# kcat/openal-soft

Measured on AMD Instinct MI355X. Metric: mixed voices/sec @48kHz 1024-sample update, HRTF stereo; fraction of HBM roofline, higher is better.
Workload: dtype f32

## Files before the change

include/oalgpu.h:

```cpp
#ifndef OALGPU_H
#define OALGPU_H

#include <stddef.h>
#include <stdint.h>

#ifdef __cplusplus
extern "C" {
#endif
#if defined(__GNUC__)
#pragma GCC visibility push(default)
#endif

#define OALGPU_BUFFER_LINE_SIZE 1024
#define OALGPU_MAX_RESAMPLER_PADDING 48
#define OALGPU_MAX_RESAMPLER_EDGE 24
#define OALGPU_HRTF_HISTORY_LENGTH 64
#define OALGPU_HRIR_LENGTH 128
#define OALGPU_MAX_SENDS 6
#define OALGPU_MAX_OUTPUT_CHANNELS 32
#define OALGPU_MAX_AMBI_CHANNELS 25
#define OALGPU_MIXER_FRAC_BITS 16

typedef enum oalgpu_error {
    OALGPU_OK = 0,
// ... 47 lines not shown
    float sf;
    uint32_t m, l;
    uint32_t filter_offset;
} oalgpu_interp_state;
int oalgpu_prepare_resampler(int resampler, uint32_t increment, oalgpu_interp_state *out);

typedef struct oalgpu_biquad {
    float z1, z2;
    float b0, b1, b2, a1, a2;
    float tb0, tb1, tb2, ta1, ta2;
    int32_t counter;
} oalgpu_biquad;
void oalgpu_biquad_reset(oalgpu_biquad *f);
void oalgpu_biquad_set_params_from_slope(oalgpu_biquad *f, int type, float f0norm, float gain,
    float slope);

int oalgpu_resample(int device, int mode, int resampler, uint32_t increment, const float *src,
    size_t srclen, uint32_t frac, float *dst, size_t n);
int oalgpu_mix(int device, const float *in, size_t n, float *out, size_t nlines,
    float *current_gains, const float *target_gains, size_t counter, size_t outpos);
int oalgpu_mix_hrtf(int device, int mode, const float *in, float *accum, uint32_t irsize,
    const float *coeffs, const uint32_t delay[2], float gain, float gainstep, size_t n);
int oalgpu_mix_hrtf_blend(int device, int mode, const float *in, float *accum, uint32_t irsize,
    const float *oldcoeffs, const uint32_t olddelay[2], float oldgain, const float *newcoeffs,
    const uint32_t newdelay[2], float newgainstep, size_t n);
typedef struct oalgpu_splitter { float coeff, lp_z1, lp_z2, ap_z1; } oalgpu_splitter;
void oalgpu_splitter_init(oalgpu_splitter *s, float f0norm);
int oalgpu_mix_direct_hrtf(int device, int mode, float *left, float *right, const float *in,
    size_t nch, float *accum, oalgpu_splitter *splitters, const float *hfscales,
    const float *chan_coeffs, size_t irsize, size_t n);
int oalgpu_biquad_dual_process(int device, oalgpu_biquad *f0, oalgpu_biquad *f1, const float *src,
    float *dst, size_t n);

typedef struct oalgpu_context oalgpu_context;

typedef struct oalgpu_context_desc {
    int32_t  device;
    int32_t  math_mode;
    uint32_t sample_rate;
    uint32_t num_dry_channels;
    uint32_t num_real_channels;
    uint32_t num_aux_sends;
    uint32_t num_slots;
    uint32_t wet_channels;
    int32_t  hrtf;
    uint32_t max_voices;
    uint32_t max_buffers;
    uint32_t voices_per_group;
    uint32_t flags;
} oalgpu_context_desc;
#define OALGPU_CTX_FIR_VALU 1u
#define OALGPU_CTX_PROFILE  2u
#define OALGPU_CTX_STREAM_ROWS 8u
#define OALGPU_CTX_APPLY_IN_VOICE_KERNEL 16u
#define OALGPU_CTX_FUSED_REDUCE 32u
#define OALGPU_CTX_RESIDENT 64u
#define OALGPU_CTX_SLICE_LINES 128u
#define OALGPU_CTX_WAVE_PAIRS 256u
#define OALGPU_CTX_ROW_SLICES 512u
#define OALGPU_CTX_SERIAL   4u

int  oalgpu_context_create(const oalgpu_context_desc *desc, oalgpu_context **out);
void oalgpu_context_destroy(oalgpu_context *ctx);

int oalgpu_hrtf_load_mhr(oalgpu_context *ctx, const void *data, size_t size);
int oalgpu_hrtf_load_store(oalgpu_context *ctx, uint32_t sample_rate, uint32_t ir_size, const float *field_distance,
    const uint8_t *field_evcount, uint32_t num_fields, const uint16_t *elev_azcount, const uint16_t *elev_iroffset,
    uint32_t num_elevs, const float *coeffs, const uint8_t *delays, uint32_t num_irs);
typedef struct oalgpu_hrtf_info {
    uint32_t sample_rate, ir_size, num_fields, num_elevs, num_irs;
} oalgpu_hrtf_info;
int oalgpu_hrtf_info_get(oalgpu_context *ctx, oalgpu_hrtf_info *out);
int oalgpu_hrtf_raw(oalgpu_context *ctx, float *field_distance, uint8_t *field_evcount,
    uint16_t *elev_azcount, uint16_t *elev_iroffset, float *coeffs, uint8_t *delays);
int oalgpu_hrtf_get_coeffs(oalgpu_context *ctx, const float *dirs, size_t count, float *coeffs,
    uint32_t *delays);
int oalgpu_set_direct_hrtf(oalgpu_context *ctx, const float *chan_coeffs ,
    const float *hfscales, float xover_norm, uint32_t irsize);
int oalgpu_set_direct_hrtf_from_store(oalgpu_context *ctx, const float *points, const float *matrix, uint32_t num_points,
    const float *order_hf_gain, float xover_freq, uint32_t ir_size, int per_hrir_min);
int oalgpu_hrtf_parse_host(const void *mhr, size_t size, uint32_t device_rate, oalgpu_hrtf_info *info, float *coeffs, uint8_t *delays);
int oalgpu_hrtf_blend_host(const void *mhr, size_t size, uint32_t device_rate, const float *dirs, size_t count,
    uint32_t *idx, float *w, float *pass, uint32_t *delays);
int oalgpu_hrtf_build_direct_host(const void *mhr, size_t size, uint32_t device_rate, uint32_t ir_size, int per_hrir_min,
    const float *points, const float *matrix, uint32_t num_points, uint32_t num_chans, float xover_freq, const float *order_hf_gain,
    float *out_coeffs, float *out_hfscales, float *out_xover_norm, uint32_t *out_irsize);

int oalgpu_buffer_register(oalgpu_context *ctx, const void *data, int fmt_type,
    uint32_t frame_step, uint32_t sample_len, uint32_t loop_start, uint32_t loop_end);
int oalgpu_buffer_release(oalgpu_context *ctx, int buffer);
int oalgpu_buffer_info(oalgpu_context *ctx, int buffer, int32_t *live, int32_t *release_pending, uint32_t *references);

int oalgpu_buffer_channel_view(oalgpu_context *ctx, int buffer, uint32_t channel);

typedef struct oalgpu_voice_desc {
    int32_t  buffer;
    int32_t  looping;
    int32_t  position;
    uint32_t position_frac;
    uint32_t frequency;
} oalgpu_voice_desc;
int oalgpu_voice_init(oalgpu_context *ctx, uint32_t voice, const oalgpu_voice_desc *desc);
int oalgpu_context_set_nfc(oalgpu_context *ctx, float w1, const uint32_t channels_per_order[5]);
int oalgpu_voice_set_nfc(oalgpu_context *ctx, uint32_t voice, float w0);

int oalgpu_voice_set_ambi_scale(oalgpu_context *ctx, uint32_t voice, float xover_norm, float hf_scale,
    float lf_scale);

typedef struct oalgpu_filter_params {
    int32_t active;
    float gain_hf, hf_norm;
    float gain_lf, lf_norm;
} oalgpu_filter_params;

typedef struct oalgpu_voice_params {
    uint32_t step;
    int32_t  resampler;
    oalgpu_filter_params direct_filter;
    float    dry_gains[OALGPU_MAX_OUTPUT_CHANNELS];
    float    hrtf_ev, hrtf_az, hrtf_dist, hrtf_spread;
    float    hrtf_gain;
    int32_t  send_slot[OALGPU_MAX_SENDS];
    oalgpu_filter_params send_filter[OALGPU_MAX_SENDS];
    float    send_gains[OALGPU_MAX_SENDS][OALGPU_MAX_AMBI_CHANNELS];
} oalgpu_voice_params;
#define OALGPU_HRTF_KEEP_TARGET (-1.0f)
int oalgpu_voice_set_hrtf_targets(oalgpu_context *ctx, const uint32_t *voices, const float *coeffs, const uint32_t *delays,
    const float *gains, size_t count);

typedef struct oalgpu_voice_pan {
    float dir[3];
    float spread;
    float dry_gain;
    float send_gain[OALGPU_MAX_SENDS];
} oalgpu_voice_pan;
int oalgpu_context_set_ambi_map(oalgpu_context *ctx, const uint8_t *index, const float *scale);
int oalgpu_slot_set_ambi_map(oalgpu_context *ctx, uint32_t slot, const uint8_t *index, const float *scale);
int oalgpu_voice_set_pan(oalgpu_context *ctx, const uint32_t *voices, const oalgpu_voice_pan *pans, size_t count);

int oalgpu_buffer_queue_link(oalgpu_context *ctx, int buffer, int next_buffer);
int oalgpu_voice_init_queue(oalgpu_context *ctx, uint32_t voice, int first_buffer, int looping, int32_t position,
    uint32_t position_frac);
int oalgpu_voice_queue_state(oalgpu_context *ctx, uint32_t voice, int32_t *current_buffer, uint32_t *buffers_done);
int oalgpu_voice_queue_unqueue(oalgpu_context *ctx, uint32_t voice, uint32_t count);

typedef int32_t (*oalgpu_callback_fn)(void *userptr, void *data, int32_t num_bytes);
int oalgpu_voice_init_callback(oalgpu_context *ctx, uint32_t voice, int fmt_type, uint32_t position_frac,
    oalgpu_callback_fn fn, void *userptr);
typedef struct oalgpu_callback_state {
    int32_t position;
    uint32_t position_frac, num_blocks, block_offset;
    int32_t stopped, play_state, has_buffer;
} oalgpu_callback_state;
int oalgpu_voice_callback_state(oalgpu_context *ctx, uint32_t voice, oalgpu_callback_state *out);

enum oalgpu_adpcm_type { OALGPU_ADPCM_IMA4 = 0, OALGPU_ADPCM_MS = 1 };
int oalgpu_buffer_register_adpcm(oalgpu_context *ctx, const void *data, int adpcm_type, uint32_t channels,
    uint32_t samples_per_block, uint32_t sample_len, uint32_t loop_start, uint32_t loop_end);

int oalgpu_voice_set_start_delay(oalgpu_context *ctx, uint32_t voice, uint32_t samples);

int oalgpu_voice_set_params(oalgpu_context *ctx, const uint32_t *voices,
    const oalgpu_voice_params *params, size_t count);
typedef struct oalgpu_param_block oalgpu_param_block;
int  oalgpu_param_block_create(oalgpu_context *ctx, const uint32_t *voices,
    const oalgpu_voice_params *params, size_t count, oalgpu_param_block **out);
// ... 329 lines not shown
```

openal-soft_amd/csrc/api_hrtf.hip:

```cpp
#include "api_context.hpp"

static uint32_t ChooseWave16(const oalgpu_context *c, const DeviceLayout &T)
{
    const bool want16 = !(c->desc.flags & OALGPU_CTX_WAVE_PAIRS) && Wave16Applies(T)
        && (T.numSends == 0 || !(c->desc.flags & (OALGPU_CTX_STREAM_ROWS | OALGPU_CTX_PROFILE)));
    if(!want16) return 0u;
    if(!c->desc.voices_per_group) return Wave16WavesFor(T.numVoices, DeviceComputeUnits(c->desc.device));
    for(uint32_t w : {4u, 8u, 16u})
        if((T.numVoices + w - 1u) / w <= c->groupsAllocated) return w;
    return 0u;
}

static int InstallHrtfData(oalgpu_context *c, HrtfData &&parsed)
{
    if(parsed.sampleRate != c->desc.sample_rate) ResampleHrtfData(parsed, c->desc.sample_rate);
    DeviceLayout T = c->L;
    T.irSize = parsed.irSize;
    T.irStride = (parsed.irSize + 15u) & ~15u;
    const bool toStreamRows = T.accLines && WaveKernelAccLines(T) == 0;
    if(toStreamRows) T.accLines = 0;
    if(c->useWave)
    {
        T.wave16 = ChooseWave16(c, T);
        if(std::max<uint32_t>(1u, WaveKernelGroups(T)) > c->groupsAllocated)
            return Fail(OALGPU_ERR_INVALID, "internal: the voice kernel's grid outgrew the partial buses");
    }
    if(int rc = oalgpu_sync(c)) return rc;
    c->hrtfHost = std::move(parsed);
    const HrtfData &h = c->hrtfHost;
    HIP_TRY(c->hFieldDist.alloc(h.fieldDistance.size())); HIP_TRY(c->hFieldDist.upload(h.fieldDistance.data(), h.fieldDistance.size()));
    HIP_TRY(c->hEvCount.alloc(h.fieldEvCount.size())); HIP_TRY(c->hEvCount.upload(h.fieldEvCount.data(), h.fieldEvCount.size()));
    HIP_TRY(c->hAzCount.alloc(h.elevAzCount.size())); HIP_TRY(c->hAzCount.upload(h.elevAzCount.data(), h.elevAzCount.size()));
    HIP_TRY(c->hIrOffset.alloc(h.elevIrOffset.size())); HIP_TRY(c->hIrOffset.upload(h.elevIrOffset.data(), h.elevIrOffset.size()));
    HIP_TRY(c->hCoeffs.alloc(h.coeffs.size())); HIP_TRY(c->hCoeffs.upload(h.coeffs.data(), h.coeffs.size()));
    HIP_TRY(c->hDelays.alloc(h.delays.size())); HIP_TRY(c->hDelays.upload(h.delays.data(), h.delays.size()));
    HrtfStoreDev &d = c->hrtfDev;
    d.irSize = h.irSize; d.numFields = uint32_t(h.fieldDistance.size()); d.numElevs = uint32_t(h.elevAzCount.size());
    d.numIrs = h.numIrs();
    d.fieldDistance = c->hFieldDist.p; d.fieldEvCount = c->hEvCount.p; d.elevAzCount = c->hAzCount.p;
    d.elevIrOffset = c->hIrOffset.p; d.coeffs = c->hCoeffs.p; d.delays = c->hDelays.p;
    c->hrtfLoaded = true;
    ++c->hrtfGeneration;

    DeviceLayout &L = c->L;
    L.hrirs = c->hCoeffs.p;
    L.irSize = h.irSize;
    L.irStride = T.irStride;
    if(L.hrtf)
    {
        const size_t n = size_t{L.numVoices} * L.irStride * 2;
        HIP_TRY(c->hrtfOld.alloc(n)); HIP_TRY(c->hrtfOld.zero()); L.hrtfOld = c->hrtfOld.p;
        HIP_TRY(c->hrtfTgt.alloc(n)); HIP_TRY(c->hrtfTgt.zero()); L.hrtfTgt = c->hrtfTgt.p;
        if(!c->directSet) c->dIrSize = h.irSize;
    }
    if(toStreamRows)
    {
        L.accLines = 0;
        if(int rc = AllocStreamRows(c)) return rc;
    }
    if(c->useWave)
    {
        L.wave16 = T.wave16;
        if(L.wave16 && L.numSends)
        {
            L.accLines = 0;
            if(!L.streams) { if(int rc = AllocStreamRows(c)) return rc; }
        }
        const uint32_t groups = std::max<uint32_t>(1u, WaveKernelGroups(L));
        L.numGroups = groups; L.numLineGroups = groups;
        if(L.wave16 && (L.wave16 != 16u || L.numSends)) c->res.enabled = false;
    }
    return OALGPU_OK;
}

int oalgpu_hrtf_load_mhr(oalgpu_context *c, const void *data, size_t size)
{
    if(!c || !data) return Fail(OALGPU_ERR_INVALID, "null argument");
    if(int rc = UseCtx(c)) return rc;
    HrtfData parsed;
    const std::string err = ParseMhr(data, size, parsed);
    if(!err.empty()) return Fail(OALGPU_ERR_INVALID, "mhr: " + err);
    return InstallHrtfData(c, std::move(parsed));
}
// ... 73 lines not shown
}

int oalgpu_set_direct_hrtf(oalgpu_context *c, const float *chan_coeffs, const float *hfscales, float xover_norm,
    uint32_t irsize)
{
    if(!c || !chan_coeffs || !hfscales || irsize < 8 || irsize > kHrirLen) return Fail(OALGPU_ERR_INVALID, "oalgpu_set_direct_hrtf: bad arguments");
    if(int rc = UseCtx(c)) return rc;
    const uint32_t nd = c->L.numDry;
    std::vector<SplitterState> sp(nd);
    for(auto &s : sp) { s.coeff = SplitterCoeff(xover_norm); s.lpZ1 = s.lpZ2 = s.apZ1 = 0.0f; }
    if(int rc = oalgpu_sync(c)) return rc;
    HIP_TRY(c->dSplit.upload(sp.data(), nd));
    HIP_TRY(c->dSplit2.upload(sp.data(), nd));
    c->dSplitCur = 0;
    c->dSplitCoeff = SplitterCoeff(xover_norm); c->runPowerSeg = 0;
    HIP_TRY(c->dHfScale.upload(hfscales, nd));
    {
        std::vector<float> cc(chan_coeffs, chan_coeffs + size_t{nd} * kHrirLen * 2);
        const uint32_t live = (irsize + 1u) & ~1u;
        for(uint32_t ch = 0; ch < nd; ++ch)
            for(uint32_t k = live; k < uint32_t(kHrirLen); ++k) { cc[(size_t{ch} * kHrirLen + k) * 2] = 0.0f; cc[(size_t{ch} * kHrirLen + k) * 2 + 1] = 0.0f; }
        HIP_TRY(c->dCoeffs.upload(cc.data(), cc.size()));
    }
    c->dIrSize = irsize;
    c->directSet = true;
    return OALGPU_OK;
}

int oalgpu_set_direct_hrtf_from_store(oalgpu_context *c, const float *points, const float *matrix, uint32_t num_points,
    const float *order_hf_gain, float xover_freq, uint32_t ir_size, int per_hrir_min)
{
    if(!c || !points || !matrix || !order_hf_gain || num_points == 0 || c->L.numDry > 16)
        return Fail(OALGPU_ERR_INVALID, "oalgpu_set_direct_hrtf_from_store: bad arguments");
    if(!c->hrtfLoaded) return Fail(OALGPU_ERR_NO_HRTF, "oalgpu_set_direct_hrtf_from_store: no data set loaded");
    const DirectHrtfBuild b = BuildDirectHrtf(c->hrtfHost, ir_size ? ir_size : c->hrtfHost.irSize, per_hrir_min != 0, points, matrix,
        num_points, c->L.numDry, xover_freq, order_hf_gain);
    return oalgpu_set_direct_hrtf(c, b.coeffs.data(), b.hfScale.data(), b.xoverNorm, std::max<uint32_t>(b.irSize, 8u));
}

int oalgpu_hrtf_parse_host(const void *mhr, size_t size, uint32_t device_rate, oalgpu_hrtf_info *info, float *coeffs, uint8_t *delays)
{
    if(!mhr || !info) return Fail(OALGPU_ERR_INVALID, "null argument");
    HrtfData h;
    const std::string err = ParseMhr(mhr, size, h);
    if(!err.empty()) return Fail(OALGPU_ERR_INVALID, "mhr: " + err);
    if(device_rate) ResampleHrtfData(h, device_rate);
    info->sample_rate = h.sampleRate; info->ir_size = h.irSize; info->num_fields = uint32_t(h.fieldDistance.size());
    info->num_elevs = uint32_t(h.elevAzCount.size()); info->num_irs = h.numIrs();
    if(coeffs) std::memcpy(coeffs, h.coeffs.data(), h.coeffs.size() * sizeof(float));
    if(delays) std::memcpy(delays, h.delays.data(), h.delays.size());
    return OALGPU_OK;
}

HrtfStoreDev HostStoreView(const HrtfData &h)
{
    HrtfStoreDev st{};
    st.irSize = h.irSize; st.numFields = uint32_t(h.fieldDistance.size());
    st.numElevs = uint32_t(h.elevAzCount.size()); st.numIrs = h.numIrs();
    st.fieldDistance = h.fieldDistance.data(); st.fieldEvCount = h.fieldEvCount.data();
    st.elevAzCount = h.elevAzCount.data(); st.elevIrOffset = h.elevIrOffset.data();
    st.coeffs = h.coeffs.data(); st.delays = h.delays.data();
    return st;
}

int oalgpu_hrtf_blend_host(const void *mhr, size_t size, uint32_t device_rate, const float *dirs, size_t count,
    uint32_t *idx, float *w, float *pass, uint32_t *delays)
{
    if(!mhr || !dirs || !idx || !w || !pass || !delays) return Fail(OALGPU_ERR_INVALID, "null argument");
    HrtfData h;
    const std::string err = ParseMhr(mhr, size, h);
    if(!err.empty()) return Fail(OALGPU_ERR_INVALID, "mhr: " + err);
    if(device_rate) ResampleHrtfData(h, device_rate);
    const HrtfStoreDev store = HostStoreView(h);
    for(size_t i = 0; i < count; ++i)
    {
        const HrirBlend b = HrtfBlendFor(store, dirs[4 * i], dirs[4 * i + 1], dirs[4 * i + 2], dirs[4 * i + 3]);
        for(int k = 0; k < 4; ++k) { idx[4 * i + k] = b.idx[k]; w[4 * i + k] = b.w[k]; }
        pass[i] = b.passthru;
        delays[2 * i] = b.delay[0]; delays[2 * i + 1] = b.delay[1];
    }
    return OALGPU_OK;
}

int oalgpu_hrtf_build_direct_host(const void *mhr, size_t size, uint32_t device_rate, uint32_t ir_size, int per_hrir_min,
    const float *points, const float *matrix, uint32_t num_points, uint32_t num_chans, float xover_freq, const float *order_hf_gain,
    float *out_coeffs, float *out_hfscales, float *out_xover_norm, uint32_t *out_irsize)
{
    if(!mhr || !points || !matrix || !order_hf_gain || !out_coeffs || !out_hfscales || num_chans < 1 || num_chans > 16 || num_points == 0)
        return Fail(OALGPU_ERR_INVALID, "oalgpu_hrtf_build_direct_host: bad arguments");
    HrtfData h;
    const std::string err = ParseMhr(mhr, size, h);
    if(!err.empty()) return Fail(OALGPU_ERR_INVALID, "mhr: " + err);
    if(device_rate) ResampleHrtfData(h, device_rate);
    const DirectHrtfBuild b = BuildDirectHrtf(h, ir_size ? ir_size : h.irSize, per_hrir_min != 0, points, matrix, num_points,
        num_chans, xover_freq, order_hf_gain);
    std::memcpy(out_coeffs, b.coeffs.data(), b.coeffs.size() * sizeof(float));
    std::memcpy(out_hfscales, b.hfScale.data(), b.hfScale.size() * sizeof(float));
    if(out_xover_norm) *out_xover_norm = b.xoverNorm;
    if(out_irsize) *out_irsize = b.irSize;
    return OALGPU_OK;
}
```

openal-soft_amd/csrc/voice_wave16.hip:

```cpp
#define OALGPU_WAVE_NO_LAUNCHER
#include "voice_wave.hip"

#pragma clang fp contract(off)

namespace oalgpu {
namespace {

constexpr int kW16Outs = kLine / 64;

constexpr int kW16Rd = 1184;
constexpr int kW16Rd2 = kMaxEdge + kPre * 64 + 8;
constexpr int kW16Area = kResampleDataSize + kLine;
static_assert(kW16Rd % 64 == 32 && kW16Rd >= kMaxPad + kPre * 64 + 8, "rd2 sits half the banks away from rd");
static_assert(kW16Rd + kW16Rd2 <= kW16Area, "the twice-parked window fits");
static_assert(kResampleDataSize >= kLine + 64, "a send's filter scan parks the unfiltered samples in the window's area");
constexpr int kW16DumpF2 = 64 * 17 + 68;
static_assert(kW16DumpF2 * 2 <= kW16Area, "the dump fits");
struct W16PhaseB {
    uint32_t xh[2][kXhDw];
    uint32_t hr[2][kHrDw];
    uint32_t hro[2][kHrDw];
    float in0[2 * kHist];
};
static_assert(sizeof(W16PhaseB) <= size_t(kW16Area) * 4, "phase B fits the area (nothing of it is written before the sample line is back in registers)");
struct alignas(16) W16Lds {
    union {
        struct { float rd[kW16Rd]; float rd2[kW16Rd2]; } a;
        struct { float rd[kResampleDataSize]; float smp[kLine]; } g;
        W16PhaseB b;
        f2 dump[kW16DumpF2];
        float raw[kW16Area];
    };
    int32_t best;
    uint32_t pad[3];
};
template<int WAVES>
struct W16Wg {
    alignas(16) f2 tabF[12 * 32];
    f2 tabP[12 * 32];
    uint32_t tabKey, tabM, tabL, pad;
    uint32_t res[12];
    W16Lds w[WAVES];
};
static_assert(sizeof(W16Wg<16>) <= 157440, "123 LDS granules: the post-process (4) and the reduction (1) fit beside it");

struct W16GenView { float *rd, *in, *rd2; int32_t &best; uint32_t *pad; };

template<int M, bool DUAL>
__device__ __forceinline__ void ResampleRingRegs(const f2 *tabF, const f2 *tabP, const float *rdb, uint32_t frac0, uint32_t increment,
    uint32_t bdst, float (&outs)[kW16Outs], uint32_t lane, const float *rd2b, uint32_t rdbIndex)
{
    constexpr int NP = (M / 2 >= 6) ? 6 : M / 2;
    constexpr int G = (M / 2) / NP;
    f2 F[2][NP], P[2][NP], S[2][NP];
    const uint32_t tstep = 64u * increment;
    const uint32_t tlast = frac0 + (bdst - 1u) * increment;
    auto load = [&](int set, uint32_t tt, int g)
    {
        tt = tt < tlast ? tt : tlast;
        const uint32_t pi = (tt >> 11) & 31u;
        const f2 *tf = tabF + pi, *tp = tabP + pi;
        const uint32_t pos = tt >> kFracBits;
#pragma unroll
        for(int q = 0; q < NP; ++q)
        {
            F[set][q] = tf[(g * NP + q) * 32];
            P[set][q] = tp[(g * NP + q) * 32];
        }
        if constexpr (DUAL)
        {
            const bool odd = ((rdbIndex + pos) & 1u) != 0u;
            const f2 *sp = reinterpret_cast<const f2*>(odd ? rd2b + pos - 1u : rdb + pos);
#pragma unroll
            for(int q = 0; q < NP; ++q) S[set][q] = sp[g * NP + q];
        }
        else
        {
            const float *s = rdb + pos;
#pragma unroll
            for(int q = 0; q < NP; ++q) S[set][q] = f2{s[2 * (g * NP + q)], s[2 * (g * NP + q) + 1]};
        }
    };
    const uint32_t tb = frac0 + lane * increment;
    load(0, tb, 0);
#pragma unroll
    for(int j = 0; j < kW16Outs; ++j)
    {
        outs[j] = 0.0f;
        if(uint32_t(64 * j) < bdst)
        {
            const uint32_t tt0 = tb + uint32_t(j) * tstep;
            const uint32_t tt = tt0 < tlast ? tt0 : tlast;
            const f2 pf = splat(float(tt & 2047u) * (1.0f / 2048.0f));
            f2 r0 = {0.0f, 0.0f}, r1 = {0.0f, 0.0f};
#pragma unroll
            for(int g = 0; g < G; ++g)
            {
                const int u = j * G + g, nx = u + 1;
                if(nx < kW16Outs * G) load(nx & 1, tb + uint32_t(nx / G) * tstep, nx % G);
#pragma unroll
                for(int q = 0; q < NP; ++q)
                {
                    const f2 c = pkfma(pf, P[u & 1][q], F[u & 1][q]);
                    if(q & 1) r1 = pkfma(c, S[u & 1][q], r1);
                    else r0 = pkfma(c, S[u & 1][q], r0);
                }
            }
            outs[j] = (r0.x + r0.y) + (r1.x + r1.y);
        }
    }
}

template<int TILES, bool LOW8>
__device__ __forceinline__ void FirMfmaEar(f4 (&acc)[5], const uint32_t (&xh)[2][kXhDw], const uint32_t (&hr)[2][kHrDw], float inv, uint32_t lane)
{
    const uint32_t i = lane & 15u, g = lane >> 4;
    const uint32_t u0 = 16u - i + 8u * g, shift = (u0 & 1u) * 2u, ud = u0 >> 1;
    const f4 vinv = {inv, inv, inv, inv};
    h8 A[2][3];
#pragma unroll
    for(int s = 0; s < 2; ++s)
#pragma unroll
        for(int c = 0; c < 3; ++c)
        {
            const uint32_t *p = hr[s] + ud + 16 * c;
            const uint32_t q0 = p[0], q1 = p[1], q2 = p[2], q3 = p[3], q4 = p[4];
            const u4 q = {__builtin_amdgcn_alignbyte(q1, q0, shift), __builtin_amdgcn_alignbyte(q2, q1, shift),
                __builtin_amdgcn_alignbyte(q3, q2, shift), __builtin_amdgcn_alignbyte(q4, q3, shift)};
            A[s][c] = __builtin_bit_cast(h8, q);
        }
#pragma unroll
    for(int T = 0; T < TILES; ++T)
    {
        __builtin_amdgcn_sched_barrier(0);
        const uint32_t j = (T == 4 && i > 3u) ? 3u : i;
        h8 B[2][3];
#pragma unroll
        for(int s = 0; s < 2; ++s)
        {
            const u4 *p = reinterpret_cast<const u4*>(xh[s]) + 32 * T + 2u * j + g;
#pragma unroll
            for(int c = 0; c < 3; ++c) B[s][c] = __builtin_bit_cast(h8, p[4 * c]);
        }
        f4 ta = {0.0f, 0.0f, 0.0f, 0.0f}, tb = ta, tc = ta;
#pragma unroll
        for(int c = 0; c < 3; ++c)
        {
            ta = __builtin_amdgcn_mfma_f32_16x16x32_f16(A[1][c], B[0][c], ta, 0, 0, 0);
            tb = __builtin_amdgcn_mfma_f32_16x16x32_f16(A[0][c], B[1][c], tb, 0, 0, 0);
            tc = __builtin_amdgcn_mfma_f32_16x16x32_f16(A[0][c], B[0][c], tc, 0, 0, 0);
        }
        f4 sum = __builtin_elementwise_fma((ta + tb) + tc, vinv, acc[T]);
        asm volatile("" : "+v"(sum));
        if(!LOW8 || i < 8u) acc[T] = sum;
        __builtin_amdgcn_sched_barrier(0);
    }
}

__device__ __forceinline__ float W16ReadLaneF(float v, int l)
{ return __builtin_bit_cast(float, __builtin_amdgcn_readlane(__builtin_bit_cast(int, v), l)); }

__device__ __forceinline__ float W16StageResponse(uint32_t (&hr)[2][kHrDw], float h, uint32_t lane)
{
    float sh, inv;
    HalfScale(WaveMaxBits(__builtin_bit_cast(uint32_t, __builtin_fabsf(h))), sh, inv);
    uint32_t hi, lo;
    SplitHalf2(h * sh, 0.0f, hi, lo);
    uint32_t *hz32 = &hr[0][0];
    for(uint32_t k = lane; k < uint32_t(2 * kHrDw); k += 64) hz32[k] = 0u;
    uint16_t *hz = reinterpret_cast<uint16_t*>(&hr[0][0]);
    const uint32_t u = 80u - lane;
    hz[0 * kHrHalves + u] = uint16_t(hi); hz[1 * kHrHalves + u] = uint16_t(lo);
    return __builtin_bit_cast(float, __builtin_amdgcn_readfirstlane(__builtin_bit_cast(int, inv)));
}

__device__ __forceinline__ uint32_t W16VoiceOf(uint32_t group, uint32_t wave, uint32_t waves)
{
    const uint32_t a = wave >> 2, b = wave & 3u;
    return group * waves + 4u * a + ((a + b) & 3u);
}

struct Next16 { const ParamRecord *recs; const int32_t *map; const float *rows; ResidentArgs res; };
struct W16Sends {
    BiquadSlot *sfilt; const float *sendTgt; float *sendCur; float *streams; uint32_t *lineGains;
    uint32_t numSends, wetCh, lineStride, spv;
};

template<bool PROF, int WAVES, bool SENDS = false, bool RES = false>
__global__ void OALGPU_SINGLE_DS_OPS __launch_bounds__(WAVES * 64) VoiceWave16Kernel(WaveArgsHrtf L, uint32_t samplesToDo, Next16 next, WaveProf prof, W16Sends S)
{
    unsigned long long tEntry = 0;
    if constexpr (PROF) tEntry = __builtin_readcyclecounter();
    constexpr uint32_t kW16Waves = uint32_t(WAVES), kW16Threads = uint32_t(WAVES) * 64u;
    __shared__ W16Wg<WAVES> sm;
    const uint32_t t = threadIdx.x;
    uint32_t lane = t & 63u;
    const uint32_t wave = __builtin_amdgcn_readfirstlane(t >> 6);
    const uint32_t group = blockIdx.x;
    const uint32_t irStride = L.irStride;
    uint32_t N = samplesToDo;
    W16Lds &w = sm.w[wave];
    asm volatile("; argument block resident" :: "s"(L.tables), "s"(L.buffers), "s"(L.ctl), "s"(L.prev), "s"(L.dfilt), "s"(L.hrtfOld),
        "s"(L.hrtfTgt), "s"(L.hist), "s"(L.ambi), "s"(L.startDelay), "s"(L.queueDone), "s"(L.partHrtf), "s"(L.hrirs),
        "s"(next.recs), "s"(next.map), "s"(L.numVoices), "s"(L.irStride), "s"(L.pad), "s"(samplesToDo));

    const uint32_t vRaw = W16VoiceOf(group, wave, kW16Waves);
    const bool haveVoice = vRaw < L.numVoices;
    const uint32_t lastVoice = L.numVoices - 1u;
    const uint32_t v = haveVoice ? vRaw : lastVoice;
    const uint32_t keyVoice = group * uint32_t(kW16Waves);

    uint32_t upd = 0u, updBase = 0u;
    if constexpr (RES)
    {
        const ResidentArgs &RA = next.res;
        upd = updBase = RA.base;
        if(t == 0)
        {
            const uint32_t old = __hip_atomic_fetch_add(RA.counters + 16u * kRcStarted, 1u, __ATOMIC_RELAXED, __HIP_MEMORY_SCOPE_AGENT);
            if(old + 1u == RA.startedTarget)
                __hip_atomic_store(RA.hostFlags + 16u * kRhResident, RA.launchId, __ATOMIC_RELAXED, __HIP_MEMORY_SCOPE_SYSTEM);
        }
    }
    for(;;)
    {
    uint32_t tU = threadIdx.x;
    if constexpr (RES) { asm volatile("" : "+v"(tU)); lane = tU & 63u; }
    const uint32_t t = tU;
    if constexpr (RES)
    {
        const ResidentArgs &RA = next.res;
        if(t == 0)
        {
            const unsigned long long tTop = __builtin_amdgcn_s_memrealtime();
            uint32_t go = 0u, fault = 0u;
            unsigned long long recs = 0ull, map = 0ull, rowsP = 0ull;
            uint32_t smp = 0u;
            if(upd != RA.endSeq)
            {
                const ResidentDoor *door = RA.door;
                const uint32_t *exitp = &door->exitSeq[RA.launchId & 3u];
                const uint32_t *rr = RA.counters + 16u * kRcRedRead;
                const bool needRed = int32_t(upd - kResidentSets) >= 0;
                const uint32_t want = (upd - kResidentSets + 1u) * RA.redPerUpdate;
                unsigned long long t0 = 0ull;
                uint32_t waitedFor = 0u;
                for(uint32_t spins = 0;; ++spins)
                {
                    const uint32_t ex = ResLoadSys(exitp), sq = ResLoadSys(&door->seq), rd = needRed ? ResLoadDev(rr) : want;
                    if(int32_t(ex - upd) <= 0) break;
                    const bool rung = int32_t(sq - upd) > 0, redOk = int32_t(rd - want) >= 0;
                    if(rung && redOk) { go = 1u; break; }
                    if(spins == 0u) { t0 = __builtin_amdgcn_s_memrealtime(); waitedFor = rung ? 2u : 1u; }
                    else if((spins & 15u) == 15u && __builtin_amdgcn_s_memrealtime() - t0 > kResidentWatchdogTicks)
                    {
                        fault = 1u;
// ... 337 lines not shown
                        for(int j = 0; j < kW16Outs; ++j) outs[j] = bak[lane + 64u * uint32_t(j)];
                        __builtin_amdgcn_sched_barrier(0);
                    }
                    else doPair(sfC, slots, false);
                }
                float stC = 0.0f, scC = 0.0f;
                if(lane < wetCh) { stC = S.sendTgt[vs * wetCh + lane]; scC = S.sendCur[vs * wetCh + lane]; }
                const uint32_t base = uint32_t(slot) * wetCh;
                const bool mine = lane >= base && lane < base + wetCh;
                float tg = 0.0f, cu = 0.0f;
                float *curp = S.sendCur + vs * wetCh + (lane - base);
                {
                    const float tgS = __shfl(stC, int(lane - base)), cuS = __shfl(scC, int(lane - base));
                    if(mine)
                    {
                        tg = playing ? tgS : 0.0f;
                        cu = counter ? cuS : tg;
                    }
                }
                const MixLineGain g = PrepareMixLine(cu, tg, counter, N);
                if(mine) *curp = g.newCur;
                if(sendFilter)
                {
                    RowLineGain r;
                    if(mine) r.add(g);
                    float *dst = rowsV + size_t{2u + si} * kLine;
#pragma unroll
                    for(int j = 0; j < kW16Outs; ++j)
                    {
                        const uint32_t k = lane + 64u * uint32_t(j);
                        dst[k] = (k < N) ? w.g.smp[k] : 0.0f;
                    }
                    StoreRowBlock(blkS, ls, lane, r, true);
                    WaveSync();
                }
                else
                {
                    if(mine) row0.add(g);
                    row0Live = true;
                    if(lane == 0) blkS[3u * ls] = 0u;
                }
            }
            if(row0Live)
            {
#pragma unroll
                for(int j = 0; j < kW16Outs; ++j) rowsV[lane + 64u * uint32_t(j)] = outs[j];
            }
            StoreRowBlock(blkV, ls, lane, row0, row0Live);
            WaveSync();
        }

        {
            const bool directFilter = (head.flags & kFlagDirectFilter) != 0;
            BiquadSlot *slots = &L.dfilt[size_t{v} * 2];
            if(directFilter)
            {
                toLine();
                doPair(fstv, slots, true);
                fromLine();
            }
            else doPair(fstv, slots, false);
        }

        stamp(2);
        __builtin_amdgcn_s_setprio(0);
        {
            const uint32_t q = N + lane;
            float hv;
            if(N == uint32_t(kLine)) hv = outs[kW16Outs - 1];
            else
            {
                const uint32_t k = q - uint32_t(kHist);
                const uint32_t j0 = (N - uint32_t(kHist)) >> 6;
                float lo = 0.0f, hi2 = 0.0f;
#pragma unroll
                for(int j = 0; j < kW16Outs; ++j) { if(uint32_t(j) == j0) lo = outs[j]; if(uint32_t(j) == j0 + 1u) hi2 = outs[j]; }
                const float sLo = __shfl(lo, int(k & 63u)), sHi = __shfl(hi2, int(k & 63u));
                const float smpv = (N >= uint32_t(kHist)) ? (((k >> 6) == j0) ? sLo : sHi) : __shfl(outs[0], int(k & 63u));
                const float old = __shfl(histv, int(q & 63u));
                hv = (q >= uint32_t(kHist)) ? smpv : old;
            }
            if(playing) __builtin_nontemporal_store(hv, &L.hist[size_t{v} * kHist + lane]);
        }
        w.b.in0[lane] = histv;
        w.b.in0[kHist + lane] = outs[0];

        const float targetGain = tail.tgtGain * (playing ? 1.0f : 0.0f);
        const float oldGain = counter ? tail.oldGain : tail.tgtGain;
        float blendGain = targetGain;
        if(counter)
        {
            fademix = N < counter ? N : counter;
            if(counter > fademix)
                blendGain = lerpf(oldGain, targetGain, float(fademix) / float(counter));
        }
        const float newStep = fademix ? blendGain / float(fademix) : 0.0f;
        gainAfterBlend = fademix ? blendGain : oldGain;
        todo = N - fademix;
        endGain = targetGain;
        if(todo && counter > N)
            endGain = lerpf(gainAfterBlend, targetGain, float(todo) / float(counter - fademix));
        const float mainStep = todo ? (endGain - gainAfterBlend) / float(todo) : 0.0f;
        const bool oldOn = fademix && oldGain > kGainSilence;
        const bool newOn = fademix && newStep * float(fademix) > kGainSilence;
        const float oldStep = fademix ? oldGain / float(fademix) : 0.0f;
        const bool merged = !dirty;
        const bool oldPass = !merged && oldOn;
        const f2 hO = (oldPass && lane < irStride) ? reinterpret_cast<const f2*>(L.hrtfOld + size_t{v} * irStride * 2)[lane] : f2{0.0f, 0.0f};
        const float gbase = gainAfterBlend - mainStep * float(fademix);
        auto gainAt = [&](uint32_t i, bool mayFade)
        {
            float g = __builtin_fmaf(mainStep, float(i), gbase);
            if(mayFade && i < fademix)
            {
                float gf = newOn ? newStep * float(i) : 0.0f;
                if(merged && oldOn) gf += oldStep * float(fademix - i);
                g = gf;
            }
            return g;
        };
        WaveSync();
        stamp2(0);

        float sx, invX;
        {
            float mxo = __builtin_fabsf(histv);
#pragma unroll
            for(int j = 0; j < kW16Outs; ++j) mxo = __builtin_fmaxf(__builtin_fabsf(outs[j]), mxo);
            const float mxw = __builtin_bit_cast(float, WaveMaxBits(__builtin_bit_cast(uint32_t, mxo)));
            const float gmax = __builtin_fmaxf(__builtin_fmaxf(__builtin_fabsf(blendGain) + __builtin_fabsf(oldGain), __builtin_fabsf(gainAfterBlend)),
                __builtin_fabsf(endGain));
            HalfScale(__builtin_bit_cast(uint32_t, mxw * gmax), sx, invX);
            invX = __builtin_bit_cast(float, __builtin_amdgcn_readfirstlane(__builtin_bit_cast(int, invX)));
            sx = __builtin_bit_cast(float, __builtin_amdgcn_readfirstlane(__builtin_bit_cast(int, sx)));
        }
        const float step64 = mainStep * 64.0f * sx;
        auto buildEar = [&](uint32_t d, auto fullTag)
        {
            constexpr bool FULL = decltype(fullTag)::value;
            if(lane < 32u) { w.b.xh[0][lane] = 0u; w.b.xh[1][lane] = 0u; }
            for(uint32_t dw = 32u + (N >> 1) + lane; dw < uint32_t(kXhDw); dw += 64u) { w.b.xh[0][dw] = 0u; w.b.xh[1][dw] = 0u; }
            WaveSync();
            uint16_t *xz = reinterpret_cast<uint16_t*>(&w.b.xh[0][0]) + 64u + lane + d;
            if(lane < d)
            {
                const float headP = (lane < N) ? w.b.in0[kHist - d + lane] * gainAt(lane, true) : 0.0f;
                uint32_t hi, lo;
                SplitHalf2(headP * sx, 0.0f, hi, lo);
                uint16_t *xh0 = reinterpret_cast<uint16_t*>(&w.b.xh[0][0]) + 64u + lane;
                xh0[0] = uint16_t(hi); xh0[kXhHalves] = uint16_t(lo);
            }
            const uint32_t i00 = lane + d;
            const float g0s = gainAt(i00, true) * sx;
            const float gls = __builtin_fmaf(mainStep, float(i00), gbase) * sx;
#pragma unroll
            for(int j = 0; j < kW16Outs; j += 2)
            {
                const float ga = (j == 0) ? g0s : __builtin_fmaf(step64, float(j), gls);
                const float gb = __builtin_fmaf(step64, float(j + 1), gls);
                float p0 = outs[j] * ga, p1 = outs[j + 1] * gb;
                if(!FULL || j + 2 == kW16Outs)
                {
                    if(i00 + 64u * uint32_t(j) >= N) p0 = 0.0f;
                    if(i00 + 64u * uint32_t(j + 1) >= N) p1 = 0.0f;
                }
                uint32_t hi, lo;
                SplitHalf2(p0, p1, hi, lo);
                xz[64 * j] = uint16_t(hi); xz[kXhHalves + 64 * j] = uint16_t(lo);
                xz[64 * (j + 1)] = uint16_t(hi >> 16); xz[kXhHalves + 64 * (j + 1)] = uint16_t(lo >> 16);
            }
        };

#pragma unroll
        for(int e = 0; e < 2; ++e)
        {
            const uint32_t d = tail.tgtDelay[e];
            if(N == uint32_t(kLine)) buildEar(d, std::true_type{}); else buildEar(d, std::false_type{});
            uint16_t *xz = reinterpret_cast<uint16_t*>(&w.b.xh[0][0]);
            if(e == 0) stamp2(1);
            const float invH = W16StageResponse(w.b.hr, e == 0 ? hT.x : hT.y, lane);
            WaveSync();
            if(e == 0) stamp2(2);
            FirMfmaEar<5, false>(accM[e], w.b.xh, w.b.hr, invX * invH, lane);
            if(e == 0) stamp2(3);
            if(oldPass)
            {
                const uint32_t od = tail.oldDelay[e];
                float xo = 0.0f;
                if(lane < fademix) xo = w.b.in0[kHist - od + lane] * (oldStep * float(fademix - lane));
                float sxo, invXo;
                HalfScale(WaveMaxBits(__builtin_bit_cast(uint32_t, __builtin_fabsf(xo))), sxo, invXo);
                invXo = __builtin_bit_cast(float, __builtin_amdgcn_readfirstlane(__builtin_bit_cast(int, invXo)));
                uint32_t hi, lo;
                SplitHalf2(xo * sxo, 0.0f, hi, lo);
                WaveSync();
                xz[0 * kXhHalves + 64u + lane] = uint16_t(hi); xz[1 * kXhHalves + 64u + lane] = uint16_t(lo);
                if(lane < 40u) { w.b.xh[0][64u + lane] = 0u; w.b.xh[1][64u + lane] = 0u; }
                const float invHO = W16StageResponse(w.b.hro, e == 0 ? hO.x : hO.y, lane);
                WaveSync();
                FirMfmaEar<1, true>(accM[e], w.b.xh, w.b.hro, invXo * invHO, lane);
            }
            WaveSync();
            stamp(3 + e);
        }
    }

    if(active)
    {
        if(dirty && (counter == 0 || fademix))
        {
            if(lane < irStride) reinterpret_cast<f2*>(L.hrtfOld + size_t{v} * irStride * 2)[lane] = hT;
        }
        if(lane == 0)
        {
            VoiceCtl &c = L.ctl[v];
            if(counter == 0 || fademix) { c.hrtfOldDelay[0] = tail.tgtDelay[0]; c.hrtfOldDelay[1] = tail.tgtDelay[1]; }
            c.hrtfOldGain = todo ? endGain : gainAfterBlend;
            uint32_t flags = (head.flags | kFlagFading) & ~kFlagDelayed;
            if(counter == 0 || fademix) flags &= ~kFlagHrtfDirty;
            c.flags = flags;
            if(!playing) c.playState = OALGPU_VOICE_STOPPED;
            else
            {
                int32_t bufPosInt = head.position;
                uint32_t bufPosFrac = head.positionFrac + head.step * (N - outPos);
                const uint32_t samplesDone = bufPosFrac >> kFracBits;
                bufPosInt = AddSat(bufPosInt, int32_t(samplesDone));
                bufPosFrac &= kFracMask;
                if(bufferItem >= 0 && bufPosInt > 0 && (head.flags & kFlagQueue))
                {
                    uint32_t buffersDone = 0;
                    const int32_t before = bufferItem;
                    AdvanceQueue(L.buffers, bufferItem, head.loopBuffer, bufPosInt, buffersDone);
                    if(buffersDone) L.queueDone[v] += buffersDone;
                    if(bufferItem >= 0 && bufferItem != before) c.buf = L.buffers[bufferItem];
                }
                else if(bufferItem >= 0 && bufPosInt > 0)
                {
                    if(looping)
                    {
                        uint32_t pos = uint32_t(bufPosInt);
                        if(pos >= buf.loopEnd)
                        {
                            pos = ((pos - buf.loopStart) % (buf.loopEnd - buf.loopStart)) + buf.loopStart;
                            bufPosInt = int32_t(pos);
                        }
                    }
                    else if(uint32_t(bufPosInt) >= buf.sampleLen)
                        bufferItem = -1;
                }
                c.position = bufPosInt;
                c.positionFrac = bufPosFrac;
                c.curBuffer = bufferItem;
                if(bufferItem < 0)
                {
                    c.loopBuffer = -1;
                    c.playState = OALGPU_VOICE_STOPPING;
                }
            }
        }
    }

    if(!RES && next.map && haveVoice)
    {
        __builtin_amdgcn_fence(__ATOMIC_RELEASE, "workgroup");
        if(next.rows && irStride <= 64u) InstallPair(L, next.map, next.recs, next.rows, v, v, false, lane);
        else
        {
            const int32_t ri = __builtin_amdgcn_readfirstlane(next.map[v]);
            if(ri >= 0) ApplyNextRecord(L, next.recs[ri], lane);
        }
    }
    stamp(5);
    {
        WaveSync();
        f2 *dump = w.dump;
        const uint32_t jc = lane & 15u, q4 = lane >> 4;
#pragma unroll
        for(int T = 0; T < 4; ++T)
#pragma unroll
            for(int r = 0; r < 4; ++r)
                dump[17u * (16u * uint32_t(T) + jc) + 4u * q4 + uint32_t(r)] = f2{accM[0][T][r], accM[1][T][r]};
        if(jc < 4u)
// ... 104 lines not shown
```

Measured before the change: 115.0 million.

## Split HRTF FIR delay into 8-aligned rows and advanced response to share staging

Each ear's delay d is decomposed as 8q - a. The coarse part q becomes a row offset into a single shared zero-padded sample array, and the fine part a is folded into an advanced copy of the response. Sample rows that do not depend on the delay are written once for both ears when the gain is constant, instead of rebuilding the whole delayed line per ear. Both ears' responses are staged up front, and the old-pass input gets its own small buffer. This adds DPP/perm packing, extra LDS zeroing and a host debug helper, and it is more complex to keep correct at the buffer edges.

```diff
diff --git a/include/oalgpu.h b/include/oalgpu.h
--- a/include/oalgpu.h
+++ b/include/oalgpu.h
@@ -153,6 +153,7 @@
 int oalgpu_hrtf_parse_host(const void *mhr, size_t size, uint32_t device_rate, oalgpu_hrtf_info *info, float *coeffs, uint8_t *delays);
 int oalgpu_hrtf_blend_host(const void *mhr, size_t size, uint32_t device_rate, const float *dirs, size_t count,
     uint32_t *idx, float *w, float *pass, uint32_t *delays);
+int oalgpu_fir_split_host(uint32_t d0, uint32_t d1, uint32_t samples, int ramp, uint32_t *out);
 int oalgpu_hrtf_build_direct_host(const void *mhr, size_t size, uint32_t device_rate, uint32_t ir_size, int per_hrir_min,
     const float *points, const float *matrix, uint32_t num_points, uint32_t num_chans, float xover_freq, const float *order_hf_gain,
     float *out_coeffs, float *out_hfscales, float *out_xover_norm, uint32_t *out_irsize);
diff --git a/openal-soft_amd/csrc/api_hrtf.hip b/openal-soft_amd/csrc/api_hrtf.hip
--- a/openal-soft_amd/csrc/api_hrtf.hip
+++ b/openal-soft_amd/csrc/api_hrtf.hip
@@ -1,4 +1,5 @@
 #include "api_context.hpp"
+#include "fir_split.hpp"
 
 static uint32_t ChooseWave16(const oalgpu_context *c, const DeviceLayout &T)
 {
@@ -238,6 +239,33 @@
     return OALGPU_OK;
 }
 
+int oalgpu_fir_split_host(uint32_t d0, uint32_t d1, uint32_t samples, int ramp, uint32_t *out)
+{
+    if(!out || d0 > 63u || d1 > 63u || samples == 0u || samples > uint32_t(kLine)) return Fail(OALGPU_ERR_INVALID, "oalgpu_fir_split_host: bad arguments");
+    const uint32_t d[2] = {d0, d1}, dmax = d0 > d1 ? d0 : d1;
+    out[0] = uint32_t(kZPad); out[1] = uint32_t(kZHalves); out[2] = uint32_t(kZRespHalves); out[3] = uint32_t(kZPairs);
+    for(int e = 0; e < 2; ++e)
+    {
+        const uint32_t q = FirSplitQ(d[e]), a = FirSplitA(d[e]);
+        out[4 + e] = q; out[6 + e] = a;
+        out[8 + e] = FirSplitU(a, 0u);
+        out[10 + e] = 8u * FirSplitBRow(q, 0u, 0u, 0u, 0u);
+    }
+    out[12] = FirSplitAHalf(0u, 0u, 0u);
+    uint32_t mask = 0u;
+    for(uint32_t k = 0; k < uint32_t(kZPairs); ++k) if(FirSplitPairPerEar(k, samples, dmax, ramp != 0)) mask |= 1u << k;
+    out[13] = mask;
+    out[14] = FirSplitZ(0);
+    out[15] = 8u * (FirSplitBRow(0u, 1u, 0u, 0u, 0u) - FirSplitBRow(0u, 0u, 0u, 0u, 0u));
+    out[16] = 8u * (FirSplitBRow(0u, 0u, 1u, 0u, 0u) - FirSplitBRow(0u, 0u, 0u, 0u, 0u));
+    out[17] = 8u * (FirSplitBRow(0u, 0u, 0u, 1u, 0u) - FirSplitBRow(0u, 0u, 0u, 0u, 0u));
+    out[18] = 8u * (FirSplitBRow(0u, 0u, 0u, 0u, 1u) - FirSplitBRow(0u, 0u, 0u, 0u, 0u));
+    out[19] = FirSplitAHalf(0u, 0u, 0u) - FirSplitAHalf(1u, 0u, 0u);
+    out[20] = FirSplitAHalf(0u, 1u, 0u) - FirSplitAHalf(0u, 0u, 0u);
+    out[21] = FirSplitAHalf(0u, 0u, 1u) - FirSplitAHalf(0u, 0u, 0u);
+    return OALGPU_OK;
+}
+
 int oalgpu_hrtf_build_direct_host(const void *mhr, size_t size, uint32_t device_rate, uint32_t ir_size, int per_hrir_min,
     const float *points, const float *matrix, uint32_t num_points, uint32_t num_chans, float xover_freq, const float *order_hf_gain,
     float *out_coeffs, float *out_hfscales, float *out_xover_norm, uint32_t *out_irsize)
diff --git a/openal-soft_amd/csrc/fir_split.hpp b/openal-soft_amd/csrc/fir_split.hpp
--- /dev/null
+++ b/openal-soft_amd/csrc/fir_split.hpp
@@ -0,0 +1,35 @@
+#pragma once
+#include <cstdint>
+
+#if defined(__HIPCC__) || defined(__CUDACC__)
+#define OALGPU_FS_HD __host__ __device__
+#else
+#define OALGPU_FS_HD
+#endif
+
+namespace oalgpu {
+
+constexpr int kZPad = 128;
+constexpr int kZHalves = 64 + kZPad + 1024 + 16;
+constexpr int kZDw = kZHalves / 2;
+constexpr int kZRespHalves = 120;
+constexpr int kZPairs = 9;
+static_assert(kZDw % 4 == 0 && kZPad % 8 == 0, "16-byte rows");
+
+OALGPU_FS_HD constexpr uint32_t FirSplitQ(uint32_t d) { return (d + 7u) >> 3; }
+OALGPU_FS_HD constexpr uint32_t FirSplitA(uint32_t d) { return 8u * FirSplitQ(d) - d; }
+OALGPU_FS_HD constexpr uint32_t FirSplitZ(int32_t m) { return uint32_t(int32_t(kZPad) + m); }
+OALGPU_FS_HD constexpr uint32_t FirSplitU(uint32_t a, uint32_t t) { return 80u + a - t; }
+OALGPU_FS_HD constexpr uint32_t FirSplitBRow(uint32_t q, uint32_t T, uint32_t j, uint32_t c, uint32_t g)
+{ return uint32_t(kZPad / 8 - 8) - q + 32u * T + 2u * j + g + 4u * c; }
+OALGPU_FS_HD constexpr uint32_t FirSplitAHalf(uint32_t i, uint32_t c, uint32_t g) { return 16u - i + 8u * g + 32u * c; }
+OALGPU_FS_HD constexpr bool FirSplitPairPerEar(uint32_t k, uint32_t N, uint32_t dmax, bool all)
+{ return all || k == 0u || (64u * (2u * k - 1u) < N && 128u * k + 63u + dmax >= N); }
+
+static_assert(FirSplitQ(63) == 8 && FirSplitA(63) == 1 && FirSplitQ(0) == 0 && FirSplitA(0) == 0 && FirSplitA(57) == 7, "d = 8 q - a");
+static_assert(FirSplitBRow(8, 0, 0, 0, 0) == 0, "the lowest read is the array's first row");
+static_assert((FirSplitBRow(0, 4, 3, 2, 3) + 1) * 8 <= uint32_t(kZHalves), "the highest read is inside the array");
+static_assert(FirSplitU(7, 0) < 112 && FirSplitAHalf(0, 2, 3) + 8 <= 112, "the advanced response stays inside r[u], u < 112");
+static_assert(FirSplitZ(64 * 16) + 64 <= uint32_t(kZHalves), "row 16 (zeros) is inside the tail pad");
+
+}
diff --git a/openal-soft_amd/csrc/voice_wave16.hip b/openal-soft_amd/csrc/voice_wave16.hip
--- a/openal-soft_amd/csrc/voice_wave16.hip
+++ b/openal-soft_amd/csrc/voice_wave16.hip
@@ -1,5 +1,6 @@
 #define OALGPU_WAVE_NO_LAUNCHER
 #include "voice_wave.hip"
+#include "fir_split.hpp"
 
 #pragma clang fp contract(off)
 
@@ -16,12 +17,16 @@
 static_assert(kResampleDataSize >= kLine + 64, "a send's filter scan parks the unfiltered samples in the window's area");
 constexpr int kW16DumpF2 = 64 * 17 + 68;
 static_assert(kW16DumpF2 * 2 <= kW16Area, "the dump fits");
+constexpr int kXoDw = (64 + 64 + 80) / 2;
 struct W16PhaseB {
-    uint32_t xh[2][kXhDw];
-    uint32_t hr[2][kHrDw];
+    uint32_t z[2][kZDw];
+    uint32_t hr[2][2][kHrDw];
     uint32_t hro[2][kHrDw];
+    uint32_t xo[2][kXoDw];
     float in0[2 * kHist];
 };
+static_assert(kXoDw % 4 == 0, "16-byte rows");
+static_assert(kZHalves == kXhHalves + 64 && kZRespHalves == kHrHalves, "fir_split.hpp restates dev_wave.hpp's sizes");
 static_assert(sizeof(W16PhaseB) <= size_t(kW16Area) * 4, "phase B fits the area (nothing of it is written before the sample line is back in registers)");
 struct alignas(16) W16Lds {
     union {
@@ -112,10 +117,10 @@
 }
 
 template<int TILES, bool LOW8>
-__device__ __forceinline__ void FirMfmaEar(f4 (&acc)[5], const uint32_t (&xh)[2][kXhDw], const uint32_t (&hr)[2][kHrDw], float inv, uint32_t lane)
+__device__ __forceinline__ void FirMfmaEar(f4 (&acc)[5], const uint32_t *x, uint32_t partDw, uint32_t row0, const uint32_t (&hr)[2][kHrDw], float inv, uint32_t lane)
 {
     const uint32_t i = lane & 15u, g = lane >> 4;
-    const uint32_t u0 = 16u - i + 8u * g, shift = (u0 & 1u) * 2u, ud = u0 >> 1;
+    const uint32_t u0 = FirSplitAHalf(i, 0u, g), shift = (u0 & 1u) * 2u, ud = u0 >> 1;
     const f4 vinv = {inv, inv, inv, inv};
     h8 A[2][3];
 #pragma unroll
@@ -133,12 +138,12 @@
     for(int T = 0; T < TILES; ++T)
     {
         __builtin_amdgcn_sched_barrier(0);
-        const uint32_t j = (T == 4 && i > 3u) ? 3u : i;
+        const uint32_t j = LOW8 ? (i & 7u) : ((T == 4 && i > 3u) ? 3u : i);
         h8 B[2][3];
 #pragma unroll
         for(int s = 0; s < 2; ++s)
         {
-            const u4 *p = reinterpret_cast<const u4*>(xh[s]) + 32 * T + 2u * j + g;
+            const u4 *p = reinterpret_cast<const u4*>(x + uint32_t(s) * partDw) + row0 + 32 * T + 2u * j + g;
 #pragma unroll
             for(int c = 0; c < 3; ++c) B[s][c] = __builtin_bit_cast(h8, p[4 * c]);
         }
@@ -172,6 +177,21 @@
     const uint32_t u = 80u - lane;
     hz[0 * kHrHalves + u] = uint16_t(hi); hz[1 * kHrHalves + u] = uint16_t(lo);
     return __builtin_bit_cast(float, __builtin_amdgcn_readfirstlane(__builtin_bit_cast(int, inv)));
+}
+
+__device__ __forceinline__ void W16StageResponses(uint32_t (&hr)[2][2][kHrDw], f2 h, uint32_t a0, uint32_t a1, uint32_t lane, float &inv0, float &inv1)
+{
+    float sh0, sh1;
+    HalfScale(WaveMaxBits(__builtin_bit_cast(uint32_t, __builtin_fabsf(h.x))), sh0, inv0);
+    HalfScale(WaveMaxBits(__builtin_bit_cast(uint32_t, __builtin_fabsf(h.y))), sh1, inv1);
+    uint32_t hi, lo;
+    SplitHalf2(h.x * sh0, h.y * sh1, hi, lo);
+    uint16_t *hz = reinterpret_cast<uint16_t*>(&hr[0][0][0]);
+    const uint32_t ua = FirSplitU(a0, lane), ub = 2u * kHrHalves + FirSplitU(a1, lane);
+    hz[ua] = uint16_t(hi); hz[kHrHalves + ua] = uint16_t(lo);
+    hz[ub] = uint16_t(hi >> 16); hz[kHrHalves + ub] = uint16_t(lo >> 16);
+    inv0 = __builtin_bit_cast(float, __builtin_amdgcn_readfirstlane(__builtin_bit_cast(int, inv0)));
+    inv1 = __builtin_bit_cast(float, __builtin_amdgcn_readfirstlane(__builtin_bit_cast(int, inv1)));
 }
 
 __device__ __forceinline__ uint32_t W16VoiceOf(uint32_t group, uint32_t wave, uint32_t waves)
@@ -675,9 +695,6 @@
             }
             if(playing) __builtin_nontemporal_store(hv, &L.hist[size_t{v} * kHist + lane]);
         }
-        w.b.in0[lane] = histv;
-        w.b.in0[kHist + lane] = outs[0];
-
         const float targetGain = tail.tgtGain * (playing ? 1.0f : 0.0f);
         const float oldGain = counter ? tail.oldGain : tail.tgtGain;
         float blendGain = targetGain;
@@ -712,6 +729,15 @@
             }
             return g;
         };
+        if(oldPass) { w.b.in0[lane] = histv; w.b.in0[kHist + lane] = outs[0]; }
+        {
+            uint32_t *hz32 = &w.b.hr[0][0][0];
+            for(uint32_t k = lane; k < uint32_t(4 * kHrDw); k += 64) hz32[k] = 0u;
+            constexpr uint32_t kFront = uint32_t(kZPad - kHist) / 2u, kTail0 = uint32_t(kZPad + kLine) / 2u;
+            static_assert(kFront <= 64u && uint32_t(kZDw) - kTail0 <= 64u, "one store per pad and part");
+            if(lane < kFront) { w.b.z[0][lane] = 0u; w.b.z[1][lane] = 0u; }
+            if(lane < uint32_t(kZDw) - kTail0) { w.b.z[0][kTail0 + lane] = 0u; w.b.z[1][kTail0 + lane] = 0u; }
+        }
         WaveSync();
         stamp2(0);
 
@@ -728,53 +754,65 @@
             sx = __builtin_bit_cast(float, __builtin_amdgcn_readfirstlane(__builtin_bit_cast(int, sx)));
         }
         const float step64 = mainStep * 64.0f * sx;
-        auto buildEar = [&](uint32_t d, auto fullTag)
-        {
-            constexpr bool FULL = decltype(fullTag)::value;
-            if(lane < 32u) { w.b.xh[0][lane] = 0u; w.b.xh[1][lane] = 0u; }
-            for(uint32_t dw = 32u + (N >> 1) + lane; dw < uint32_t(kXhDw); dw += 64u) { w.b.xh[0][dw] = 0u; w.b.xh[1][dw] = 0u; }
-            WaveSync();
-            uint16_t *xz = reinterpret_cast<uint16_t*>(&w.b.xh[0][0]) + 64u + lane + d;
-            if(lane < d)
-            {
-                const float headP = (lane < N) ? w.b.in0[kHist - d + lane] * gainAt(lane, true) : 0.0f;
-                uint32_t hi, lo;
-                SplitHalf2(headP * sx, 0.0f, hi, lo);
-                uint16_t *xh0 = reinterpret_cast<uint16_t*>(&w.b.xh[0][0]) + 64u + lane;
-                xh0[0] = uint16_t(hi); xh0[kXhHalves] = uint16_t(lo);
-            }
+        const uint32_t d0 = tail.tgtDelay[0], d1 = tail.tgtDelay[1], dmax = d0 > d1 ? d0 : d1;
+        const bool ramp = (uint32_t(__builtin_amdgcn_readfirstlane(__builtin_bit_cast(int, mainStep))) << 1) != 0u;
+        uint32_t *zrow = &w.b.z[0][0] + uint32_t(kZPad - kHist) / 2u + (lane >> 1) + 32u * (lane & 1u);
+        const uint32_t zsel = (lane & 1u) ? 0x03020706u : 0x05040100u;
+        auto storePair = [&](int k, float pA, float pB)
+        {
+            uint32_t hi, lo;
+            SplitHalf2(pA, pB, hi, lo);
+            const uint32_t nh = uint32_t(__builtin_amdgcn_update_dpp(0, int(hi), 0xB1, 0xF, 0xF, true));
+            const uint32_t nl = uint32_t(__builtin_amdgcn_update_dpp(0, int(lo), 0xB1, 0xF, 0xF, true));
+            zrow[64 * k] = __builtin_amdgcn_perm(nh, hi, zsel);
+            zrow[kZDw + 64 * k] = __builtin_amdgcn_perm(nl, lo, zsel);
+        };
+        auto commonRows = [&]()
+        {
+            const float gcs = gbase * sx;
+#pragma unroll
+            for(int k = 1; k < kZPairs; ++k)
+                if(!FirSplitPairPerEar(uint32_t(k), N, dmax, false))
+                    storePair(k, outs[2 * k - 1] * gcs, (2 * k < kW16Outs) ? outs[2 * k < kW16Outs ? 2 * k : 0] * gcs : 0.0f);
+        };
+        auto earRows = [&](uint32_t d, bool all)
+        {
             const uint32_t i00 = lane + d;
             const float g0s = gainAt(i00, true) * sx;
             const float gls = __builtin_fmaf(mainStep, float(i00), gbase) * sx;
-#pragma unroll
-            for(int j = 0; j < kW16Outs; j += 2)
-            {
-                const float ga = (j == 0) ? g0s : __builtin_fmaf(step64, float(j), gls);
-                const float gb = __builtin_fmaf(step64, float(j + 1), gls);
-                float p0 = outs[j] * ga, p1 = outs[j + 1] * gb;
-                if(!FULL || j + 2 == kW16Outs)
-                {
-                    if(i00 + 64u * uint32_t(j) >= N) p0 = 0.0f;
-                    if(i00 + 64u * uint32_t(j + 1) >= N) p1 = 0.0f;
-                }
-                uint32_t hi, lo;
-                SplitHalf2(p0, p1, hi, lo);
-                xz[64 * j] = uint16_t(hi); xz[kXhHalves + 64 * j] = uint16_t(lo);
-                xz[64 * (j + 1)] = uint16_t(hi >> 16); xz[kXhHalves + 64 * (j + 1)] = uint16_t(lo >> 16);
-            }
+            {
+                const uint32_t ih = i00 - uint32_t(kHist);
+                float pH = histv * (gainAt(ih, true) * sx), p0 = outs[0] * g0s;
+                if(i00 < uint32_t(kHist) || ih >= N) pH = 0.0f;
+                if(i00 >= N) p0 = 0.0f;
+                storePair(0, pH, p0);
+            }
+#pragma unroll
+            for(int k = 1; k < kZPairs; ++k)
+                if(FirSplitPairPerEar(uint32_t(k), N, dmax, all))
+                {
+                    const int jA = 2 * k - 1, jB = 2 * k < kW16Outs ? 2 * k : 0;
+                    float pA = outs[jA] * __builtin_fmaf(step64, float(jA), gls);
+                    float pB = outs[jB] * __builtin_fmaf(step64, float(jB), gls);
+                    if(i00 + 64u * uint32_t(jA) >= N) pA = 0.0f;
+                    if(2 * k >= kW16Outs || i00 + 64u * uint32_t(jB) >= N) pB = 0.0f;
+                    storePair(k, pA, pB);
+                }
         };
 
+        float invH0, invH1;
+        W16StageResponses(w.b.hr, hT, FirSplitA(d0), FirSplitA(d1), lane, invH0, invH1);
+        if(!ramp) commonRows();
 #pragma unroll
         for(int e = 0; e < 2; ++e)
         {
-            const uint32_t d = tail.tgtDelay[e];
-            if(N == uint32_t(kLine)) buildEar(d, std::true_type{}); else buildEar(d, std::false_type{});
-            uint16_t *xz = reinterpret_cast<uint16_t*>(&w.b.xh[0][0]);
+            const uint32_t d = e == 0 ? d0 : d1;
+            earRows(d, ramp);
             if(e == 0) stamp2(1);
-            const float invH = W16StageResponse(w.b.hr, e == 0 ? hT.x : hT.y, lane);
             WaveSync();
             if(e == 0) stamp2(2);
-            FirMfmaEar<5, false>(accM[e], w.b.xh, w.b.hr, invX * invH, lane);
+            FirMfmaEar<5, false>(accM[e], &w.b.z[0][0], uint32_t(kZDw), FirSplitBRow(FirSplitQ(d), 0u, 0u, 0u, 0u), w.b.hr[e],
+                invX * (e == 0 ? invH0 : invH1), lane);
             if(e == 0) stamp2(3);
             if(oldPass)
             {
@@ -786,12 +824,14 @@
                 invXo = __builtin_bit_cast(float, __builtin_amdgcn_readfirstlane(__builtin_bit_cast(int, invXo)));
                 uint32_t hi, lo;
                 SplitHalf2(xo * sxo, 0.0f, hi, lo);
+                uint32_t *xo32 = &w.b.xo[0][0];
+                for(uint32_t k = lane; k < uint32_t(2 * kXoDw); k += 64) xo32[k] = 0u;
                 WaveSync();
-                xz[0 * kXhHalves + 64u + lane] = uint16_t(hi); xz[1 * kXhHalves + 64u + lane] = uint16_t(lo);
-                if(lane < 40u) { w.b.xh[0][64u + lane] = 0u; w.b.xh[1][64u + lane] = 0u; }
+                uint16_t *xz = reinterpret_cast<uint16_t*>(xo32) + 64u + lane;
+                xz[0] = uint16_t(hi); xz[2 * kXoDw] = uint16_t(lo);
                 const float invHO = W16StageResponse(w.b.hro, e == 0 ? hO.x : hO.y, lane);
                 WaveSync();
-                FirMfmaEar<1, true>(accM[e], w.b.xh, w.b.hro, invXo * invHO, lane);
+                FirMfmaEar<1, true>(accM[e], &w.b.xo[0][0], uint32_t(kXoDw), 0u, w.b.hro, invXo * invHO, lane);
             }
             WaveSync();
             stamp(3 + e);
```

Result: no change. 114.1 million (-0.8%).
